# razayunus/ManhattanSLAM

Measured on AMD Instinct MI355X. Metric: RGB-D frames/sec at 640x480 (ORB+surfel front end), higher is better.
Workload: dtype u8/i32 (ORB)/f32+f64 (surfel)

## Files before the change

manhattanslam_amd/csrc/msl_sf.h:

```cpp
#pragma once

#include "msl_common.h"

#include <hip/hip_ext.h>

namespace msl {
namespace sf {

constexpr int SP = 8;
constexpr int NCHUNK = 10;
constexpr double MAX_ANGLE_COS = 0.1, HUBER_RANGE = 0.4, MIN_TOLERATE_DIFF = 0.1;
constexpr unsigned T_INF = 0xFFFFFFFFu;
constexpr int PROP_ROUNDS = 6;
constexpr unsigned short IDX_NONE = 0xFFFF, IDX_PLANE = 0xFFFE;
constexpr int LIST_D = 256;
constexpr int SCAN_ITEMS = 1024;
#ifndef MSL_SUB_ITEMS
#define MSL_SUB_ITEMS 128
#endif
constexpr int SUB_ITEMS = MSL_SUB_ITEMS;
constexpr int DEFER_WIN = 32;
#ifndef MSL_FUSEREC_PLANES
#define MSL_FUSEREC_PLANES 0
#endif
__host__ __device__ inline size_t fuserec_index(int nseeds, unsigned seed, int word) {
#if MSL_FUSEREC_PLANES
    return (size_t)word * (size_t)nseeds + seed;
#else
    (void)nseeds; return 3 * (size_t)seed + (size_t)word;
#endif
}

enum SfCtr {
    CTR_LIVE = 0,
    CTR_NEW = 1,
    CTR_DELETED = 2,
    CTR_UPDATED = 3,
    CTR_BEFORE = 4,
    CTR_ERR = 5,
    CTR_AFTER = 6,
    CTR_TAIL_FLAG = 7,
    CTR_SELECTED = 7,
    CTR_TOT_NEW = 8, CTR_TOT_DELETED = 9, CTR_TOT_UPDATED = 10, CTR_TOT_KF = 11, CTR_TOT_BEFORE = 12,
    CTR_WIDE = 13,
    CTR_COUNT = 16
};

struct alignas(16) HotPk { float px, py, pz; unsigned tl; };
struct HotRec { float px, py, pz; int updateTimes, lastUpdate; };
constexpr unsigned HOT_WIDE = 0x80000000u, HOT_HOLE = 0xFFFFFFFFu;
__host__ __device__ inline bool tl_fits(int ut, int lu) { return (unsigned)ut < 2048u && ((unsigned)lu + (1u << 19)) < (1u << 20); }
__host__ __device__ inline unsigned tl_pack(int ut, int lu) { return ((unsigned)ut << 20) | ((unsigned)lu & 0xFFFFFu); }
__host__ __device__ inline int tl_ut(unsigned tl) { return (int)(tl >> 20); }
__host__ __device__ inline int tl_lu(unsigned tl) { return (int)(tl << 12) >> 12; }
struct alignas(32) ColdRec { float nx, ny, nz, size, color, weight; unsigned rgbf; unsigned _spare; };
constexpr unsigned COLD_WIDE = 1u << 24;
struct MapSoA {
    HotPk *hot;
    ColdRec *cold;
    int *rgbWide;
    int *utlWide;
    long long *wideFlag;
};
__host__ __device__ inline bool rgb_fits(int r, int g, int b) { return ((unsigned)r | (unsigned)g | (unsigned)b) < 256u; }
__host__ __device__ inline unsigned rgb_pack(int r, int g, int b) { return (unsigned)r | ((unsigned)g << 8) | ((unsigned)b << 16); }

template <typename T> using gptr = const T __attribute__((address_space(1))) *;
struct FrameDev {
    const uint8_t *gray; const float *depth; const int32_t *member;
    float pose[16], invPose[16];
    int ref, _pad;
#ifdef __HIPCC__
    __device__ __forceinline__ gptr<uint8_t> grayG() const { return (gptr<uint8_t>)gray; }
    __device__ __forceinline__ gptr<float> depthG() const { return (gptr<float>)depth; }
    __device__ __forceinline__ gptr<int32_t> memberG() const { return (gptr<int32_t>)member; }
#endif
};

struct alignas(32) AssignRec {
    float x, y, meanIntensity;
    unsigned stable;
    double invDepth;
    unsigned long long _pad;
};

struct FuseAux {
    MapSoA map;
    unsigned long long cap;
    unsigned *delU, *delUCount;
    unsigned *delList;
};
struct DeferCtl {
    long long ext[DEFER_WIN + 1];
    unsigned delCnt[DEFER_WIN];
    unsigned logBase[DEFER_WIN];
    unsigned nMoves;
    int flagStride;
    const uint8_t *candOk, *fused;
    const msl_surfel *cand;
    FuseAux aux;
};

struct SfDev {
    int W, H, spW, spH, nseeds, npx;
    float fx, fy, cx, cy, fuseFar, fuseNear;
    unsigned long long gstride, gbytes, dstride, mstride;
    unsigned gsB, dsB, msB;
    const FrameDev *frames;
    msl_seed *seeds, *seedsTmp;
    msl_surfel *cand;
    uint8_t *candOk;
    uint8_t *fused;
    uint2 *tex;
    float4 *fuseRec;
    unsigned short *index, *amap;
    unsigned *tmin;
    AssignRec *arec;
    float *pxInv;
    unsigned *wl;
    unsigned *wlCount;
    int *chunkAbort;
    int *changed;
    MapSoA map;
    unsigned long long cap;
    long long *ctr;
    msl_surfel *newSurfels;
    unsigned *blockSums, *blockUpd, *delList, *srcOf;
    unsigned *sbKeys, *deal;
    int dealG;
    unsigned *tickets;
    unsigned *delU;
    unsigned *delUCount;
    const float *colX, *rowY;
    int pxStride;
    int flagStride;
    int kf;
    int prevSlotAbs;
    DeferCtl *dc;
    unsigned *moveDst;
    unsigned long long *loc64;
    unsigned *vposD;
    unsigned *locKeys, *vposKeys;
    unsigned *dBig;
    unsigned *bitmap;
    HotPk *stageHot; ColdRec *stageCold; int *stageRgb, *stageUtl;
};

#ifdef __HIPCC__
__device__ __forceinline__ AssignRec assign_rec(const msl_seed &s) {
    AssignRec a;
    a.x = s.x; a.y = s.y; a.meanIntensity = s.meanIntensity; a.stable = s.stable ? 1u : 0u;
    a.invDepth = s.meanDepth > 0 ? 1.0 / (double)s.meanDepth : -1.0; a._pad = 0;
    return a;
}
__device__ __forceinline__ int seed_chunk(int seedI, int nseeds) {
    const int step = nseeds / NCHUNK;
    if (step == 0) return NCHUNK - 1;
    const int c = seedI / step;
    return c > NCHUNK - 1 ? NCHUNK - 1 : c;
}
template <typename T> __device__ __forceinline__ gptr<T> byte_off(gptr<T> p, unsigned off) {
    return reinterpret_cast<gptr<T>>(reinterpret_cast<const char __attribute__((address_space(1))) *>(p) + off);
}
template <typename T> __device__ __forceinline__ gptr<T> byte_off(const T *p, unsigned off) { return byte_off((gptr<T>)p, off); }
template <typename T> using gptr_w = T __attribute__((address_space(1))) *;
template <typename T> __device__ __forceinline__ gptr_w<T> byte_off_w(T *p, unsigned off) {
    return reinterpret_cast<gptr_w<T>>(reinterpret_cast<char __attribute__((address_space(1))) *>((gptr_w<T>)p) + off);
}
__device__ __forceinline__ uint8_t gray_at(const SfDev &P, const FrameDev &F, int y, int x) { return *byte_off(F.grayG(), (unsigned)y * P.gsB + (unsigned)x); }
__device__ __forceinline__ float depth_at(const SfDev &P, const FrameDev &F, int y, int x) { return *byte_off(F.depthG(), (unsigned)y * P.dsB + 4u * (unsigned)x); }
__device__ __forceinline__ int32_t member_at(const SfDev &P, const FrameDev &F, int y, int x) {
    return *byte_off(F.memberG(), ((unsigned)y >> 1) * P.msB + 4u * ((unsigned)x >> 1));
}
__device__ __forceinline__ void vec3b(const SfDev &P, const FrameDev &F, float row, float col, int &r, int &g, int &b) {
    const unsigned long long off = (unsigned long long)(int)row * P.gstride + 3ull * (unsigned long long)(int)col;
    r = off < P.gbytes ? F.grayG()[off] : 0;
    g = off + 1 < P.gbytes ? F.grayG()[off + 1] : 0;
    b = off + 2 < P.gbytes ? F.grayG()[off + 2] : 0;
}
__device__ __forceinline__ void back_project(const SfDev &P, float u, float v, float d, float &x, float &y, float &z) {
    x = (u - P.cx) / P.fx * d;
    y = (v - P.cy) / P.fy * d;
    z = d;
}
__device__ __forceinline__ float get_weight(float d) { const double a = 1.0 / (double)d / (double)d; return (float)(1.0 < a ? 1.0 : a); }
__device__ __forceinline__ void mul4(const float *m, float v0, float v1, float v2, float v3, float out[4]) {
#pragma unroll
    for (int r = 0; r < 4; r++) out[r] = ((m[r] * v0 + m[4 + r] * v1) + m[8 + r] * v2) + m[12 + r] * v3;
}
__device__ __forceinline__ void mul3(const float *m, float v0, float v1, float v2, float out[3]) {
#pragma unroll
    for (int r = 0; r < 3; r++) out[r] = (m[r] * v0 + m[4 + r] * v1) + m[8 + r] * v2;
}
#endif

template <typename T>
__host__ __device__ inline void inverse4(const T *m, T *inv) {
#define M_(r, c) m[(c) * 4 + (r)]
#define DET3(r0, r1, r2, c0, c1, c2)                                                                     \
    (M_(r0, c0) * (M_(r1, c1) * M_(r2, c2) - M_(r1, c2) * M_(r2, c1)) -                                 \
     M_(r0, c1) * (M_(r1, c0) * M_(r2, c2) - M_(r1, c2) * M_(r2, c0)) +                                 \
     M_(r0, c2) * (M_(r1, c0) * M_(r2, c1) - M_(r1, c1) * M_(r2, c0)))
    T cof[4][4];
    for (int r = 0; r < 4; r++)
        for (int c = 0; c < 4; c++) {
            int rr[3], cc[3], k = 0;
            for (int i = 0; i < 4; i++) if (i != r) rr[k++] = i;
            k = 0;
            for (int i = 0; i < 4; i++) if (i != c) cc[k++] = i;
            const T d = DET3(rr[0], rr[1], rr[2], cc[0], cc[1], cc[2]);
            cof[r][c] = ((r + c) & 1) ? -d : d;
        }
    const T det = ((M_(0, 0) * cof[0][0] + M_(0, 1) * cof[0][1]) + M_(0, 2) * cof[0][2]) + M_(0, 3) * cof[0][3];
    for (int r = 0; r < 4; r++)
        for (int c = 0; c < 4; c++) inv[c * 4 + r] = cof[c][r] / det;
#undef DET3
#undef M_
}

#ifdef __HIPCC__
__device__ __forceinline__ bool xcd_slot(int blocksPerFrame, int nSlots, int &slot, int &blk) {
    const unsigned lin = blockIdx.x;
    const unsigned j = lin >> 3;
    slot = (int)(lin & 7u) + 8 * (int)(j / (unsigned)blocksPerFrame);
    blk = (int)(j % (unsigned)blocksPerFrame);
    return slot < nSlots;
}
#endif
inline unsigned xcd_grid(int blocksPerFrame, int nSlots) { return 8u * (unsigned)((nSlots + 7) / 8) * (unsigned)blocksPerFrame; }

enum { SK_SEED_INIT = 0, SK_ASSIGN, SK_PROP, SK_COMMIT_PX, SK_UPDATE_SEEDS, SK_COMMIT_SEEDS, SK_SEED_PLANE, SK_FUSE, SK_NEW, SK_COMPACT,
       SK_CONVERT, SK_COPY };

#define MSL_SF_LAUNCH_LDS(prof, kid, st, kern, grid, block, lds, ...)                                  \
    do {                                                                                               \
        hipEvent_t _ea, _eb;                                                                           \
        if ((prof).kernel_pair(kid, &_ea, &_eb))                                                       \
            hipExtLaunchKernelGGL(kern, grid, block, lds, st, _ea, _eb, 0, __VA_ARGS__);               \
        else                                                                                           \
            hipLaunchKernelGGL(kern, grid, block, lds, st, __VA_ARGS__);                               \
    } while (0)
#define MSL_SF_LAUNCH(prof, kid, st, kern, grid, block, ...) MSL_SF_LAUNCH_LDS(prof, kid, st, kern, grid, block, 0, __VA_ARGS__)

bool sp_init_attributes(int nseeds);
void sp_launch_stage(KernelProfiler &prof, hipStream_t st, const SfDev &P, int nFrames, bool propLds);
void sp_launch_depth_u16(hipStream_t st, const void *src, size_t srcStride, size_t srcFrameStride, float *dst, size_t dstFrameStride, int W, int H, int nFrames,
                         float factor);
int sp_debug_div100(const float *x_host, double *out_host, size_t n);
int sp_debug_chain(const float *x_host, const int32_t *n_host, int lists, int huber, float *out_host);
void map_launch_fuse(KernelProfiler &prof, hipStream_t st, const SfDev &P, int slot, const FrameDev &F, int nSubGrid, int nSubHint, bool deferred, bool dealt, unsigned blkStride);
void map_launch_compact(KernelProfiler &prof, hipStream_t st, const SfDev &P, int slot, bool resident);
void map_launch_deal(hipStream_t st, const SfDev &P);
int map_debug_deal(const uint32_t *keys_host, int G, uint32_t *deal_host);
void map_launch_replay(KernelProfiler &prof, hipStream_t st, const SfDev &P, int nFrames, unsigned blkStride);
void map_launch_empty_pair(KernelProfiler &prof, hipStream_t st);
void map_launch_set_ctr(hipStream_t st, const SfDev &P, long long n, int wide);
void map_launch_add_ctr(hipStream_t st, const SfDev &P, long long add);
void map_launch_aos_to_soa(KernelProfiler &prof, hipStream_t st, const SfDev &P, const msl_surfel *src, long long n, bool atEnd);
void map_launch_soa_to_aos(KernelProfiler &prof, hipStream_t st, const SfDev &P, msl_surfel *dst, long long n);
void map_launch_select_count(hipStream_t st, const SfDev &P, int mode, int arg);
void map_launch_select_write(hipStream_t st, const SfDev &P, int mode, int arg, msl_surfel *out, int markDeleted);
void map_launch_collect_changed(hipStream_t st, const SfDev &P, int ref, long long n, unsigned *count, unsigned *idxOut, msl_surfel *recOut, unsigned capOut);
void map_launch_empty(hipStream_t st, int grid, hipEvent_t a, hipEvent_t b);

}
}
```

manhattanslam_amd/csrc/msl_sf_sp_assign.hip:

```cpp

#include "msl_sf_sp_dev.h"

namespace {

__global__ __launch_bounds__(256) void kb_seed_init(SfDev P) {
    const int slot = blockIdx.y;
    const int seedI = blockIdx.x * 256 + threadIdx.x;
    if (seedI >= P.nseeds) return;
    if (seedI == 0) P.wlCount[slot] = 0;
    const FrameDev F = P.frames[slot];
    const int spX = seedI % P.spW, spY = seedI / P.spW;
    int imageX = spX * SP + SP / 2, imageY = spY * SP + SP / 2;
    imageX = imageX < (P.W - 1) ? imageX : (P.W - 1);
    imageY = imageY < (P.H - 1) ? imageY : (P.H - 1);
    msl_seed s;
    memset(&s, 0, sizeof(s));
    P.fused[(size_t)slot * P.flagStride + seedI] = 0;
    if (member_at(P, F, imageY, imageX) != -1) {
        P.seeds[(size_t)slot * P.nseeds + seedI] = s; P.arec[(size_t)slot * P.nseeds + seedI] = assign_rec(s);
        return;
    }
    s.use = 1;
    s.x = (float)imageX; s.y = (float)imageY;
    vec3b(P, F, (float)imageY, (float)imageX, s.r, s.g, s.b);
    s.meanIntensity = gray_at(P, F, imageY, imageX);
    s.meanDepth = depth_at(P, F, imageY, imageX);
    if (s.meanDepth < 0.01) {
        int xb = spX * SP + SP / 2 - SP, yb = spY * SP + SP / 2 - SP;
        int xe = xb + SP * 2, ye = yb + SP * 2;
        xb = xb > 0 ? xb : 0; yb = yb > 0 ? yb : 0;
        xe = xe < P.W - 1 ? xe : P.W - 1; ye = ye < P.H - 1 ? ye : P.H - 1;
        bool found = false;
        for (int j = yb; j < ye && !found; j++)
            for (int i = xb; i < xe; i++) {
                const float d = depth_at(P, F, j, i);
                if (d > 0.01) { s.meanDepth = d; found = true; break; }
            }
    }
    P.seeds[(size_t)slot * P.nseeds + seedI] = s;
    P.arec[(size_t)slot * P.nseeds + seedI] = assign_rec(s);
}

constexpr int ASSIGN_NY = 2;
__global__ __launch_bounds__(256) void kb_assign(SfDev P, int it, int nSlots, int nbx, int nby) {
    const int bpr = (nbx + 3) >> 2;
    const int nbyG = (nby + ASSIGN_NY - 1) / ASSIGN_NY;
    int slot, blk;
    if (!xcd_slot(bpr * nbyG, nSlots, slot, blk)) return;
    if (blk == 0) {
        if (it > 0 && threadIdx.x < 8) P.changed[slot * 8 + threadIdx.x] = threadIdx.x == 0 ? 1 : 0;
        if (threadIdx.x >= 64 && threadIdx.x < 64 + NCHUNK) P.chunkAbort[(slot * 2 + (it & 1)) * 16 + threadIdx.x - 64] = 0x7FFFFFFF;
    }
    const int wv = __builtin_amdgcn_readfirstlane((int)(threadIdx.x >> 6));
    const int byg = blk / bpr, bxi = (blk - byg * bpr) * 4 + wv;
    if (bxi >= nbx) return;
    const int bx = bxi - 1, by0 = byg * ASSIGN_NY - 1;
    const bool okx0 = bx >= 0 && bx < P.spW, okx1 = bx + 1 < P.spW;
    const int bxc = min(bx, P.spW - 1);
    const AssignRec *arec = P.arec + (unsigned)slot * (unsigned)P.nseeds;
    AssignRec cr[ASSIGN_NY + 1][2];
    int rowIdx[ASSIGN_NY + 1];
#pragma unroll
    for (int r = 0; r <= ASSIGN_NY; r++) {
        const int rc = min(max(by0 + r, 0), P.spH - 1);
        rowIdx[r] = rc * P.spW + bx;
        const AssignRec *rp = arec + (rc * P.spW + bxc);
        cr[r][0] = rp[0]; cr[r][1] = rp[1];
    }
    const FrameDev F = P.frames[slot];
    unsigned short *index = P.index + (size_t)slot * P.pxStride, *amap = P.amap + (size_t)slot * P.pxStride;
    float *pxInv = P.pxInv + (size_t)slot * P.pxStride;
    unsigned *tmin = P.tmin + (size_t)slot * P.nseeds;
    const int lane = threadIdx.x & 63, lx = lane & 7, ly = lane >> 3;
    const int colI = 8 * bx + 4 + lx;
    const float colF = (float)colI;
    const bool colIn = colI >= 0 && colI < P.W;
    bool inImg[ASSIGN_NY];
    int mem[ASSIGN_NY], cur[ASSIGN_NY];
    float gI[ASSIGN_NY], dIn[ASSIGN_NY];
    unsigned tCur[ASSIGN_NY];
#pragma unroll
    for (int k = 0; k < ASSIGN_NY; k++) {
        const int rowI = 8 * (by0 + k) + 4 + ly;
        inImg[k] = colIn && rowI >= 0 && rowI < P.H && by0 + k + 1 < nby;
        const int rowC = min(max(rowI, 0), P.H - 1), colC = min(max(colI, 0), P.W - 1), pc = rowC * P.W + colC;
        mem[k] = member_at(P, F, rowC, colC);
        gI[k] = gray_at(P, F, rowC, colC);
        dIn[k] = it == 0 ? depth_at(P, F, rowC, colC) : *byte_off(pxInv, 4u * (unsigned)pc);
        cur[k] = it == 0 ? 0 : (int)*byte_off(index, 2u * (unsigned)pc);
    }
#pragma unroll
    for (int k = 0; k < ASSIGN_NY; k++)
        tCur[k] = it == 0 ? 0u : *byte_off(tmin, 4u * (unsigned)cur[k]);
#pragma unroll
    for (int k = 0; k < ASSIGN_NY; k++) {
        const int by = by0 + k;
        if (__ballot(inImg[k]) == 0) continue;
        const bool oky0 = by >= 0 && by < P.spH, oky1 = by + 1 < P.spH;
        const int rowI = 8 * by + 4 + ly;
        const int p = rowI * P.W + colI;
        const bool isPlane = mem[k] != -1;
        const float myIntensity = gI[k];
        float myInvDepth = dIn[k];
        if (it == 0) {
            myInvDepth = 0.0f;
            if (dIn[k] > 0.01) myInvDepth = (float)(1.0 / (double)dIn[k]);
            if (inImg[k] && !isPlane) *byte_off_w(pxInv, 4u * (unsigned)p) = myInvDepth;
        }
        const bool pxHasDepth = myInvDepth > 0;
        const double myInvD = (double)myInvDepth;
        const float rowF = (float)rowI;
        float minDistDepth = 1e6f, minDistNodepth = 1e6f;
        int minSpIndexDepth = -1, minSpIndexNodepth = -1;
        bool allHasDepth = true;
        auto consider = [&](const AssignRec &C, int spIndex, bool use) {
            float nodepthCost = 0;
            const float dist = (C.x - colF) * (C.x - colF) + (C.y - rowF) * (C.y - rowF);
            nodepthCost += dist / ((SP / 2) * (SP / 2));
            const float intensityDiff = C.meanIntensity - myIntensity;
            nodepthCost = (float)((double)nodepthCost + div100_exact((double)(intensityDiff * intensityDiff)));
            const bool has = C.invDepth >= 0 && pxHasDepth;
            const float inverseDepthDiff = (float)(C.invDepth - myInvD);
            const float withDepth = (float)((double)nodepthCost + (double)(inverseDepthDiff * inverseDepthDiff) * 400.0);
            const float depthCost = has ? withDepth : nodepthCost;
            allHasDepth = allHasDepth && (has || !use);
            const bool bd = use && depthCost < minDistDepth, bn = use && nodepthCost < minDistNodepth;
            minDistDepth = bd ? depthCost : minDistDepth; minSpIndexDepth = bd ? spIndex : minSpIndexDepth;
            minDistNodepth = bn ? nodepthCost : minDistNodepth; minSpIndexNodepth = bn ? spIndex : minSpIndexNodepth;
        };
        const bool anyStable = (cr[k][0].stable | cr[k][1].stable | cr[k + 1][0].stable | cr[k + 1][1].stable) != 0;
        if (okx0 && oky0) consider(cr[k][0], rowIdx[k], true);
        if (okx0 && oky1) consider(cr[k + 1][0], rowIdx[k + 1], ly != 0);
        if (okx1 && oky0) consider(cr[k][1], rowIdx[k] + 1, lx != 0);
        if (okx1 && oky1) consider(cr[k + 1][1], rowIdx[k + 1] + 1, lx != 0 && ly != 0);
        const int pick = allHasDepth ? minSpIndexDepth : minSpIndexNodepth;
        if (!inImg[k]) continue;
        if (it == 0) { *byte_off_w(index, 2u * (unsigned)p) = isPlane ? (unsigned short)0 : (unsigned short)(pick >= 0 ? pick : 0); continue; }
        *byte_off_w(amap, 2u * (unsigned)p) = isPlane ? IDX_PLANE : (pick >= 0 ? (unsigned short)pick : IDX_NONE);
        if (!isPlane && pick >= 0) {
            if (tCur[k] == 0) {
                if (anyStable && tmin[pick] > (unsigned)p + 1u) atomicMin(&tmin[pick], (unsigned)p + 1u);
            } else if (pick != cur[k]) {
                P.wl[(size_t)slot * P.pxStride + atomicAdd(&P.wlCount[slot], 1u)] = (unsigned)p;
            }
        }
    }
}

__device__ __forceinline__ bool relax_pixel(unsigned *tmin, const unsigned short *index, const unsigned short *amap, int p) {
    const unsigned short a = amap[p];
    if (a >= IDX_PLANE) return false;
    const unsigned tc = __hip_atomic_load(&tmin[index[p]], __ATOMIC_RELAXED, __HIP_MEMORY_SCOPE_AGENT);
    if (tc == 0 || tc > (unsigned)p) return false;
    if (__hip_atomic_load(&tmin[a], __ATOMIC_RELAXED, __HIP_MEMORY_SCOPE_AGENT) <= (unsigned)p + 1u) return false;
    return atomicMin(&tmin[a], (unsigned)p + 1u) > (unsigned)p + 1u;
}

constexpr int PROP_BLOCKS = 16;
__global__ __launch_bounds__(256) void kb_prop(SfDev P, int round, int nSlots) {
    int slot, blk;
    if (!xcd_slot(PROP_BLOCKS, nSlots, slot, blk)) return;
    if (!P.changed[slot * 8 + round]) return;
    unsigned *tmin = P.tmin + (size_t)slot * P.nseeds;
    const unsigned short *index = P.index + (size_t)slot * P.pxStride, *amap = P.amap + (size_t)slot * P.pxStride;
    const unsigned *wl = P.wl + (size_t)slot * P.pxStride;
    const unsigned nwl = P.wlCount[slot];
    bool any = false;
    for (unsigned e = blk * 256 + threadIdx.x; e < nwl; e += PROP_BLOCKS * 256) any |= relax_pixel(tmin, index, amap, (int)wl[e]);
    if (any) P.changed[slot * 8 + round + 1] = 1;
}

__global__ __launch_bounds__(1024) void kb_prop_finish(SfDev P) {
    __shared__ int s_ch;
    const int slot = blockIdx.x;
    if (threadIdx.x == 0) s_ch = P.changed[slot * 8 + PROP_ROUNDS];
    __syncthreads();
    unsigned *tmin = P.tmin + (size_t)slot * P.nseeds;
    const unsigned short *index = P.index + (size_t)slot * P.pxStride, *amap = P.amap + (size_t)slot * P.pxStride;
    const unsigned *wl = P.wl + (size_t)slot * P.pxStride;
    const unsigned nwl = P.wlCount[slot];
    while (s_ch) {
        __syncthreads();
        if (threadIdx.x == 0) s_ch = 0;
        __syncthreads();
        bool any = false;
        for (unsigned e = threadIdx.x; e < nwl; e += 1024) any |= relax_pixel(tmin, index, amap, (int)wl[e]);
        if (any) s_ch = 1;
        __syncthreads();
    }
}

constexpr int PROP_LDS_MAX_SEEDS = 36 * 1024;
__global__ __launch_bounds__(256) void kb_prop_lds(SfDev P) {
    extern __shared__ unsigned s_t[];
    const int slot = blockIdx.x;
    const unsigned nwl = P.wlCount[slot];
    if (nwl == 0) return;
    unsigned *tmin = P.tmin + (size_t)slot * P.nseeds;
    const unsigned short *index = P.index + (size_t)slot * P.pxStride, *amap = P.amap + (size_t)slot * P.pxStride;
    const unsigned *wl = P.wl + (size_t)slot * P.pxStride;
    constexpr int NT = 256, R = 16;
    unsigned ep[R];
    unsigned short ec[R], ea[R];
#pragma unroll
    for (int r = 0; r < R; r++) {
        const unsigned e = threadIdx.x + r * NT;
        ep[r] = 0xFFFFFFFFu; ec[r] = 0; ea[r] = 0;
        if (e < nwl) { const unsigned p = wl[e]; ep[r] = p; ec[r] = index[p]; ea[r] = amap[p]; }
    }
    for (int i = threadIdx.x; i < P.nseeds; i += NT) s_t[i] = tmin[i];
    __syncthreads();
    auto relax = [&](unsigned p, unsigned short cur, unsigned short a) -> bool {
        if (a >= IDX_PLANE) return false;
        const unsigned tc = s_t[cur];
        if (tc == 0 || tc > p) return false;
        if (s_t[a] <= p + 1u) return false;
        return atomicMin(&s_t[a], p + 1u) > p + 1u;
    };
    int any;
    do {
        bool ch = false;
#pragma unroll
        for (int r = 0; r < R; r++)
            if (ep[r] != 0xFFFFFFFFu) ch |= relax(ep[r], ec[r], ea[r]);
        for (unsigned e = threadIdx.x + R * NT; e < nwl; e += NT) { const unsigned p = wl[e]; ch |= relax(p, index[p], amap[p]); }
        any = __syncthreads_or(ch ? 1 : 0);
    } while (any);
    for (int i = threadIdx.x; i < P.nseeds; i += NT) {
        const unsigned t = s_t[i];
        if (t != tmin[i]) tmin[i] = t;
    }
}

__global__ __launch_bounds__(256) void kb_commit_px(SfDev P, int nSlots) {
    int slot, blk;
    if (!xcd_slot(((P.npx + 7) / 8 + 255) / 256, nSlots, slot, blk)) return;
    const int p0 = (blk * 256 + threadIdx.x) * 8;
    if (p0 >= P.npx) return;
    unsigned short *index = P.index + (size_t)slot * P.pxStride;
    const uint4 a4 = *reinterpret_cast<const uint4 *>(P.amap + (size_t)slot * P.pxStride + p0);
    uint4 i4 = *reinterpret_cast<const uint4 *>(index + p0);
    const unsigned *tmin = P.tmin + (size_t)slot * P.nseeds;
    unsigned aw[4] = {a4.x, a4.y, a4.z, a4.w}, iw[4] = {i4.x, i4.y, i4.z, i4.w};
    bool changed = false;
#pragma unroll
    for (int k = 0; k < 8; k++) {
        const unsigned a = (aw[k >> 1] >> (16 * (k & 1))) & 0xFFFFu, cur = (iw[k >> 1] >> (16 * (k & 1))) & 0xFFFFu;
        if (a >= IDX_PLANE || a == cur || p0 + k >= P.npx) continue;
        if (tmin[cur] <= (unsigned)(p0 + k)) {
            iw[k >> 1] = (iw[k >> 1] & ~(0xFFFFu << (16 * (k & 1)))) | (a << (16 * (k & 1)));
            changed = true;
        }
    }
    if (changed) { i4.x = iw[0]; i4.y = iw[1]; i4.z = iw[2]; i4.w = iw[3]; *reinterpret_cast<uint4 *>(index + p0) = i4; }
}

__global__ void k_debug_div100(const float *x, double *out, long long n) {
    const long long i = (long long)blockIdx.x * 256 + threadIdx.x;
    if (i < n) out[i] = div100_exact((double)(x[i] * x[i]));
}

}

namespace msl {
namespace sf {

bool sp_init_attributes(int nseeds) {
    if (nseeds > PROP_LDS_MAX_SEEDS) return false;
    return hipFuncSetAttribute((const void *)kb_prop_lds, hipFuncAttributeMaxDynamicSharedMemorySize, (int)(sizeof(unsigned) * PROP_LDS_MAX_SEEDS)) == hipSuccess;
}

void sp_launch_seed_init(KernelProfiler &prof, hipStream_t sp, const SfDev &P, int n) {
    MSL_SF_LAUNCH(prof, SK_SEED_INIT, sp, kb_seed_init, sp_seed_grid(P, n), dim3(256), P);
}

void sp_launch_pixel_pass(KernelProfiler &prof, hipStream_t sp, const SfDev &P, int n, int it, bool propLds) {
    const int W = P.W, H = P.H;
    const unsigned un = (unsigned)n;
    const int nbx = ((W - 5) >> 3) + 2, nby = ((H - 5) >> 3) + 2;
    const dim3 pxGrid(xcd_grid(((nbx + 3) / 4) * ((nby + ASSIGN_NY - 1) / ASSIGN_NY), n)), flatPx(xcd_grid(((P.npx + 7) / 8 + 255) / 256, n));
    MSL_SF_LAUNCH(prof, SK_ASSIGN, sp, kb_assign, pxGrid, dim3(256), P, it, n, nbx, nby);
    if (it > 0) {
        prof.begin(SK_PROP, sp);
        if (propLds) {
            hipLaunchKernelGGL(kb_prop_lds, dim3(un), dim3(256), sizeof(unsigned) * P.nseeds, sp, P);
        } else {
            for (int r = 0; r < PROP_ROUNDS; r++) hipLaunchKernelGGL(kb_prop, dim3(xcd_grid(PROP_BLOCKS, n)), dim3(256), 0, sp, P, r, n);
            hipLaunchKernelGGL(kb_prop_finish, dim3(un), dim3(1024), 0, sp, P);
        }
        prof.end(sp);
        MSL_SF_LAUNCH(prof, SK_COMMIT_PX, sp, kb_commit_px, flatPx, dim3(256), P, n);
    }
}

int sp_debug_div100(const float *x_host, double *out_host, size_t n) {
    if (n == 0) return MSL_OK;
    if (!x_host || !out_host) return MSL_ERR_INVALID;
    DevBuf x, out;
    MSL_HIP_TRY(grow_all(0, {{x, sizeof(float) * n}, {out, sizeof(double) * n}}));
    MSL_HIP_TRY(hipMemcpy(x.p, x_host, sizeof(float) * n, hipMemcpyHostToDevice));
    hipLaunchKernelGGL(k_debug_div100, dim3((unsigned)((n + 255) / 256)), dim3(256), 0, 0, (const float *)x.p, (double *)out.p, (long long)n);
    MSL_HIP_TRY(hipMemcpy(out_host, out.p, sizeof(double) * n, hipMemcpyDeviceToHost));
    return MSL_OK;
}

}
}
```

manhattanslam_amd/csrc/msl_sf_sp_seeds.hip:

```cpp

#include "msl_sf_sp_dev.h"

namespace {

struct SeedUpd {
    int state;
    int cnt, sumI, sumX, sumY;
    int depthLoop;
    float meanDepth;
};
static_assert(sizeof(SeedUpd) <= sizeof(msl_seed), "the hand-over record fits a seedsTmp record");
template <bool STRADDLE>
__global__ __launch_bounds__(256) void kb_update_seeds(SfDev P, int it, int nSlots) {
    __shared__ __attribute__((aligned(16))) float s_depth[16][272];
    int slot, blk;
    if (!xcd_slot((P.nseeds + 15) / 16, nSlots, slot, blk)) return;
#ifdef MSL_FUSE_STAMPS
    unsigned long long ust[8]; int usn = 0;
#define USTAMP() ust[usn++] = __builtin_amdgcn_s_memtime()
#else
#define USTAMP()
#endif
    USTAMP();
    const int g = threadIdx.x >> 4, l = threadIdx.x & 15;
    const int seedI = blk * 16 + g;
    const FrameDev F = P.frames[slot];
    const unsigned short *index = P.index + (size_t)slot * P.pxStride;
    msl_seed S;
    memset(&S, 0, sizeof(S));
    bool active = seedI < P.nseeds;
    bool stable = false;
    if (active) {
        S = P.seeds[(size_t)slot * P.nseeds + seedI];
        stable = it > 0 ? (P.tmin[(size_t)slot * P.nseeds + seedI] == T_INF) : (S.stable != 0);
        if (!S.use || stable) {
            if (l == 0) {
                P.seeds[(size_t)slot * P.nseeds + seedI].stable = stable;
                P.arec[(size_t)slot * P.nseeds + seedI].stable = stable ? 1u : 0u;
                reinterpret_cast<SeedUpd *>(P.seedsTmp + ((size_t)slot * P.nseeds + seedI))->state = 0;
                P.tmin[(size_t)slot * P.nseeds + seedI] = stable ? T_INF : 0u;
            }
            active = false;
        }
    }
    if (!__ballot(active)) return;
    const int spX = seedI % P.spW, spY = seedI / P.spW;
    const int xb0 = spX * SP + SP / 2 - SP, yb0 = spY * SP + SP / 2 - SP;
    const int xb = xb0 > 0 ? xb0 : 0, yb = yb0 > 0 ? yb0 : 0;
    const int xe = (xb0 + SP * 2) < P.W - 1 ? (xb0 + SP * 2) : P.W - 1, ye = (yb0 + SP * 2) < P.H - 1 ? (yb0 + SP * 2) : P.H - 1;
    int sumX = 0, sumY = 0, sumI = 0, cnt = 0, nd = 0;
    {
        const int rq = l >> 2, cq = l & 3;
        const int col0 = xb0 + 4 * cq;
        const bool quadIn = col0 >= 0 && (STRADDLE ? col0 < P.W : col0 + 3 < P.W);
        const int colc = quadIn ? (STRADDLE ? min(col0, P.W - 4) : col0) : 0;
        Quad<unsigned short> idq[4];
        Quad<float> dq[4];
        Quad<uint8_t> gq[4];
#pragma unroll
        for (int m = 0; m < 4; m++) {
            const int jc = min(max(yb0 + 4 * m + rq, 0), P.H - 1);
            idq[m] = load_quad(byte_off(index, 2u * (unsigned)(jc * P.W + colc)));
            dq[m] = load_quad(byte_off(F.depthG(), (unsigned)jc * P.dsB + 4u * (unsigned)colc));
            gq[m] = load_quad(byte_off(F.grayG(), (unsigned)jc * P.gsB + (unsigned)colc));
        }
#pragma unroll
        for (int m = 0; m < 4; m++) {
            const int j = yb0 + 4 * m + rq;
            const bool rowOk = active && quadIn && j >= yb && j < ye;
            bool hd[4];
            int c = 0;
#pragma unroll
            for (int e = 0; e < 4; e++) {
                const int col = colc + e;
                const bool own = rowOk && (!STRADDLE || col >= col0) && col >= xb && col < xe && idq[m].v[e] == seedI;
                hd[e] = own && dq[m].v[e] >= DEPTH_01_F;
                if (own) { sumX += col; sumY += j; sumI += gq[m].v[e]; cnt++; }
                c += hd[e] ? 1 : 0;
            }
            const int incl = row_incl_scan(c);
            int o = nd + incl - c;
#pragma unroll
            for (int e = 0; e < 4; e++)
                if (hd[e]) s_depth[g][o++] = dq[m].v[e];
            nd += row_lane_i32<15>(incl);
        }
    }
    USTAMP();
    sumX = row_sum_i32(sumX); sumY = row_sum_i32(sumY); sumI = row_sum_i32(sumI); cnt = row_sum_i32(cnt);
    __builtin_amdgcn_wave_barrier();
    const bool depthLoop = active && cnt != 0 && nd > 0;
    if (l == 0 && active && cnt == 0)
        atomicMin(&P.chunkAbort[(slot * 2 + (it & 1)) * 16 + seed_chunk(seedI, P.nseeds)], seedI);
    const int ndL = depthLoop ? nd : 0;
    const int nblk = rows_max_i32((ndL + 15) >> 4);
    float meanDepth = 0.0f;
    {
        float sd = 0.0f;
        for (int bq = 0; bq < nblk; bq++) {
            const int e = l + 16 * bq;
            sd = chain_block_f32(sd, e < ndL ? s_depth[g][e] : 0.0f);
        }
        const float sumDepth = row_lane_f32<15>(sd);
        if (depthLoop) meanDepth = sumDepth / (float)nd;
    }
    USTAMP();
    bool open = depthLoop;
    for (int newtonI = 0; newtonI < 5; newtonI++) {
        if (!__ballot(open)) break;
        int inr = 0;
        bool tail = false;
        for (int bq = 0; bq < nblk; bq++) {
            const int e = l + 16 * bq;
            if (open && e < ndL) {
                const float residual = meanDepth - s_depth[g][e];
                if (in_huber_band(residual)) inr++; else tail = true;
            }
        }
        inr = row_sum_i32(inr);
        const bool anyTail = __ballot(tail) != 0ull;
        float sa = 0.0f;
        for (int bq = 0; bq < nblk; bq++) {
            const int e = l + 16 * bq;
            float t = 0.0f;
            if (open && e < ndL) {
                const float residual = meanDepth - s_depth[g][e];
                if (in_huber_band(residual)) t = 2 * residual;
                else t = residual > 0 ? __builtin_inff() : -__builtin_inff();
            }
            sa = anyTail ? chain_block_huber(sa, t) : chain_block_f32(sa, t);
        }
        const float sumA = row_lane_f32<15>(sa);
        const float sumB = (float)(2 * inr);
        const float deltaDepth = (float)((double)(-sumA) / ((double)sumB + 10.0));
        if (open) {
            meanDepth = meanDepth + deltaDepth;
            if ((deltaDepth < 0.01 && deltaDepth > -0.01) || newtonI == 4) open = false;
        }
    }
    USTAMP();
    if (active && l == 0) {
        SeedUpd U;
        U.state = cnt == 0 ? 1 : 2; U.cnt = cnt; U.sumI = sumI; U.sumX = sumX; U.sumY = sumY; U.depthLoop = depthLoop ? 1 : 0; U.meanDepth = meanDepth;
        *reinterpret_cast<SeedUpd *>(P.seedsTmp + ((size_t)slot * P.nseeds + seedI)) = U;
    }
#ifdef MSL_FUSE_STAMPS
    USTAMP();
    if (slot == 0 && (threadIdx.x & 63) == 0) {
        for (int q = 1; q < usn; q++) atomicAdd(&P.delList[96 + q], (unsigned)(ust[q] - ust[q - 1]));
        atomicAdd(&P.delList[96], 1u);
    }
#endif
}

__global__ __launch_bounds__(256) void kb_commit_seeds(SfDev P, int it) {
    const int slot = blockIdx.y;
    const int seedI = blockIdx.x * 256 + threadIdx.x;
    if (seedI >= P.nseeds) return;
    if (seedI == 0) P.wlCount[slot] = 0;
    const size_t si = (size_t)slot * P.nseeds + seedI;
    const SeedUpd U = *reinterpret_cast<const SeedUpd *>(P.seedsTmp + si);
    if (U.state == 0) return;
    const int abortAt = P.chunkAbort[(slot * 2 + (it & 1)) * 16 + seed_chunk(seedI, P.nseeds)];
    if (U.state == 1 || seedI > abortAt) {
        P.seeds[si].stable = 0; P.arec[si].stable = 0u; P.tmin[si] = 0u;
        return;
    }
    const FrameDev &F = P.frames[slot];
    static_assert(sizeof(msl_seed) == 64 && offsetof(msl_seed, meanDepth) == 40 && offsetof(msl_seed, r) == 48 && offsetof(msl_seed, stable) == 61, "msl_seed layout");
    uint4 *rec = reinterpret_cast<uint4 *>(P.seeds + si);
    const uint4 w0o = rec[0], w2o = rec[2], w3o = rec[3];
    const float sumIntensityNum = (float)U.cnt;
    const float sumIntensity = (float)U.sumI / sumIntensityNum, mX = (float)U.sumX / sumIntensityNum, mY = (float)U.sumY / sumIntensityNum;
    const float preIntensity = __uint_as_float(w2o.w), preX = __uint_as_float(w0o.x), preY = __uint_as_float(w0o.y);
    int tR = 0, tG = 0, tB = 0;
    vec3b(P, F, mY, mX, tR, tG, tB);
    const float updateDiff = fabsf(preIntensity - sumIntensity) + fabsf(preX - mX) + fabsf(preY - mY);
    const bool tStable = updateDiff < 0.2;
    const float tDepth = U.depthLoop ? U.meanDepth : 0.0f;
    uint4 w0 = w0o, w2 = w2o, w3 = w3o;
    w0.x = __float_as_uint(mX); w0.y = __float_as_uint(mY);
    w2.z = __float_as_uint(tDepth); w2.w = __float_as_uint(sumIntensity);
    w3.x = (unsigned)tR; w3.y = (unsigned)tG; w3.z = (unsigned)tB;
    w3.w = (w3.w & 0x00FF00FFu) | (tStable ? 0x100u : 0u);
    rec[0] = w0; rec[2] = w2; rec[3] = w3;
    P.tmin[si] = tStable ? T_INF : 0u;
    AssignRec a;
    a.x = mX; a.y = mY; a.meanIntensity = sumIntensity; a.stable = tStable ? 1u : 0u;
    a.invDepth = tDepth > 0 ? 1.0 / (double)tDepth : -1.0; a._pad = 0;
    P.arec[si] = a;
}

__global__ __launch_bounds__(64) void k_debug_chain(const float *x, const int *n, float *out, int lists, int huber) {
    const int q = blockIdx.x * 4 + (threadIdx.x >> 4), l = threadIdx.x & 15;
    const int nq = q < lists ? n[q] : 0;
    int nblk = (nq + 15) >> 4;
#pragma unroll
    for (int d = 32; d >= 16; d >>= 1) nblk = max(nblk, __shfl_xor(nblk, d, 64));
    nblk = __builtin_amdgcn_readfirstlane(nblk);
    float s = 0.0f;
    for (int bq = 0; bq < nblk; bq++) {
        const int e = l + 16 * bq;
        const float t = e < nq ? x[(size_t)q * 256 + e] : 0.0f;
        s = huber ? chain_block_huber(s, t) : chain_block_f32(s, t);
    }
    if (q < lists && l == 15) out[q] = s;
}

}

namespace msl {
namespace sf {

void sp_launch_seed_pass(KernelProfiler &prof, hipStream_t sp, const SfDev &P, int n, int it) {
    if (sp_quad_straddles(P.W)) MSL_SF_LAUNCH(prof, SK_UPDATE_SEEDS, sp, kb_update_seeds<true>, dim3(xcd_grid((P.nseeds + 15) / 16, n)), dim3(256), P, it, n);
    else MSL_SF_LAUNCH(prof, SK_UPDATE_SEEDS, sp, kb_update_seeds<false>, dim3(xcd_grid((P.nseeds + 15) / 16, n)), dim3(256), P, it, n);
    MSL_SF_LAUNCH(prof, SK_COMMIT_SEEDS, sp, kb_commit_seeds, sp_seed_grid(P, n), dim3(256), P, it);
}

int sp_debug_chain(const float *x_host, const int32_t *n_host, int lists, int huber, float *out_host) {
    if (lists <= 0) return MSL_OK;
    if (!x_host || !n_host || !out_host) return MSL_ERR_INVALID;
    for (int q = 0; q < lists; q++) if (n_host[q] < 0 || n_host[q] > 256) return MSL_ERR_INVALID;
    DevBuf x, cnt, out;
    MSL_HIP_TRY(grow_all(0, {{x, sizeof(float) * 256 * (size_t)lists}, {cnt, sizeof(int) * (size_t)lists}, {out, sizeof(float) * (size_t)lists}}));
    MSL_HIP_TRY(hipMemcpy(x.p, x_host, sizeof(float) * 256 * (size_t)lists, hipMemcpyHostToDevice));
    MSL_HIP_TRY(hipMemcpy(cnt.p, n_host, sizeof(int) * (size_t)lists, hipMemcpyHostToDevice));
    hipLaunchKernelGGL(k_debug_chain, dim3((unsigned)((lists + 3) / 4)), dim3(64), 0, 0, (const float *)x.p, (const int *)cnt.p, (float *)out.p, lists, huber);
    MSL_HIP_TRY(hipMemcpy(out_host, out.p, sizeof(float) * (size_t)lists, hipMemcpyDeviceToHost));
    return MSL_OK;
}

}
}
```

Before: 26830.

## Retile assign rows, cache Newton depth blocks in registers, sign-bit depth test

Each assign block now covers three superpixel rows instead of two, so more neighbour records are reused per load and fewer blocks are launched. The chunkAbort init moves to threads 32..41. In the seed update, the first four 16-wide depth blocks are kept in registers across Newton iterations, and their residual terms are cached too, which cuts repeated LDS reads. The candidate depth test becomes a scalar sign-bit check on the high word of invDepth. These are separate ideas; the taller tile raises register pressure and may lower occupancy.

```diff
diff --git a/manhattanslam_amd/csrc/msl_sf.h b/manhattanslam_amd/csrc/msl_sf.h
--- a/manhattanslam_amd/csrc/msl_sf.h
+++ b/manhattanslam_amd/csrc/msl_sf.h
@@ -83,6 +83,13 @@
     double invDepth;
     unsigned long long _pad;
 };
+constexpr double arec_inv_depth(float meanDepth) { return meanDepth > 0 ? 1.0 / (double)meanDepth : -1.0; }
+static_assert(arec_inv_depth(0.0f) == -1.0 && arec_inv_depth(-0.0f) == -1.0 && arec_inv_depth(-2.5f) == -1.0 && arec_inv_depth(__builtin_nanf("")) == -1.0,
+              "no valid depth: the literal -1.0");
+static_assert(__builtin_bit_cast(unsigned long long, arec_inv_depth(__builtin_inff())) == 0ull && arec_inv_depth(2.0f) == 0.5 &&
+              arec_inv_depth(__builtin_bit_cast(float, 1u)) > 0 && arec_inv_depth(__builtin_bit_cast(float, 1u)) < 1e46,
+              "a valid depth: sign bit clear from +inf (+0.0) down to the smallest denormal (finite)");
+static_assert((__builtin_bit_cast(unsigned long long, -1.0) >> 63) == 1ull, "-1.0 has its sign bit set");
 
 struct FuseAux {
     MapSoA map;
@@ -150,8 +157,13 @@
 __device__ __forceinline__ AssignRec assign_rec(const msl_seed &s) {
     AssignRec a;
     a.x = s.x; a.y = s.y; a.meanIntensity = s.meanIntensity; a.stable = s.stable ? 1u : 0u;
-    a.invDepth = s.meanDepth > 0 ? 1.0 / (double)s.meanDepth : -1.0; a._pad = 0;
+    a.invDepth = arec_inv_depth(s.meanDepth); a._pad = 0;
     return a;
+}
+__device__ __forceinline__ bool arec_has_depth(const AssignRec &C) {
+    int hi = (int)(__builtin_bit_cast(unsigned long long, C.invDepth) >> 32);
+    asm("" : "+s"(hi));
+    return hi >= 0;
 }
 __device__ __forceinline__ int seed_chunk(int seedI, int nseeds) {
     const int step = nseeds / NCHUNK;
diff --git a/manhattanslam_amd/csrc/msl_sf_sp_assign.hip b/manhattanslam_amd/csrc/msl_sf_sp_assign.hip
--- a/manhattanslam_amd/csrc/msl_sf_sp_assign.hip
+++ b/manhattanslam_amd/csrc/msl_sf_sp_assign.hip
@@ -41,18 +41,19 @@
     P.arec[(size_t)slot * P.nseeds + seedI] = assign_rec(s);
 }
 
-constexpr int ASSIGN_NY = 2;
-__global__ __launch_bounds__(256) void kb_assign(SfDev P, int it, int nSlots, int nbx, int nby) {
-    const int bpr = (nbx + 3) >> 2;
-    const int nbyG = (nby + ASSIGN_NY - 1) / ASSIGN_NY;
+constexpr int ASSIGN_NY = 3;
+constexpr int ASSIGN_WAVES = 4;
+__host__ __device__ constexpr int assign_blocks(int nbx, int nby) { return ((nbx + ASSIGN_WAVES - 1) / ASSIGN_WAVES) * ((nby + ASSIGN_NY - 1) / ASSIGN_NY); }
+__global__ __launch_bounds__(64 * ASSIGN_WAVES) void kb_assign(SfDev P, int it, int nSlots, int nbx, int nby) {
+    const int bpr = (nbx + ASSIGN_WAVES - 1) / ASSIGN_WAVES;
     int slot, blk;
-    if (!xcd_slot(bpr * nbyG, nSlots, slot, blk)) return;
+    if (!xcd_slot(assign_blocks(nbx, nby), nSlots, slot, blk)) return;
     if (blk == 0) {
         if (it > 0 && threadIdx.x < 8) P.changed[slot * 8 + threadIdx.x] = threadIdx.x == 0 ? 1 : 0;
-        if (threadIdx.x >= 64 && threadIdx.x < 64 + NCHUNK) P.chunkAbort[(slot * 2 + (it & 1)) * 16 + threadIdx.x - 64] = 0x7FFFFFFF;
+        if (threadIdx.x >= 32 && threadIdx.x < 32 + NCHUNK) P.chunkAbort[(slot * 2 + (it & 1)) * 16 + threadIdx.x - 32] = 0x7FFFFFFF;
     }
     const int wv = __builtin_amdgcn_readfirstlane((int)(threadIdx.x >> 6));
-    const int byg = blk / bpr, bxi = (blk - byg * bpr) * 4 + wv;
+    const int byg = blk / bpr, bxi = (blk - byg * bpr) * ASSIGN_WAVES + wv;
     if (bxi >= nbx) return;
     const int bx = bxi - 1, by0 = byg * ASSIGN_NY - 1;
     const bool okx0 = bx >= 0 && bx < P.spW, okx1 = bx + 1 < P.spW;
@@ -114,12 +115,13 @@
         int minSpIndexDepth = -1, minSpIndexNodepth = -1;
         bool allHasDepth = true;
         auto consider = [&](const AssignRec &C, int spIndex, bool use) {
+            const bool candHas = arec_has_depth(C);
             float nodepthCost = 0;
             const float dist = (C.x - colF) * (C.x - colF) + (C.y - rowF) * (C.y - rowF);
             nodepthCost += dist / ((SP / 2) * (SP / 2));
             const float intensityDiff = C.meanIntensity - myIntensity;
             nodepthCost = (float)((double)nodepthCost + div100_exact((double)(intensityDiff * intensityDiff)));
-            const bool has = C.invDepth >= 0 && pxHasDepth;
+            const bool has = candHas && pxHasDepth;
             const float inverseDepthDiff = (float)(C.invDepth - myInvD);
             const float withDepth = (float)((double)nodepthCost + (double)(inverseDepthDiff * inverseDepthDiff) * 400.0);
             const float depthCost = has ? withDepth : nodepthCost;
@@ -278,8 +280,8 @@
     const int W = P.W, H = P.H;
     const unsigned un = (unsigned)n;
     const int nbx = ((W - 5) >> 3) + 2, nby = ((H - 5) >> 3) + 2;
-    const dim3 pxGrid(xcd_grid(((nbx + 3) / 4) * ((nby + ASSIGN_NY - 1) / ASSIGN_NY), n)), flatPx(xcd_grid(((P.npx + 7) / 8 + 255) / 256, n));
-    MSL_SF_LAUNCH(prof, SK_ASSIGN, sp, kb_assign, pxGrid, dim3(256), P, it, n, nbx, nby);
+    const dim3 pxGrid(xcd_grid(assign_blocks(nbx, nby), n)), flatPx(xcd_grid(((P.npx + 7) / 8 + 255) / 256, n));
+    MSL_SF_LAUNCH(prof, SK_ASSIGN, sp, kb_assign, pxGrid, dim3(64 * ASSIGN_WAVES), P, it, n, nbx, nby);
     if (it > 0) {
         prof.begin(SK_PROP, sp);
         if (propLds) {
diff --git a/manhattanslam_amd/csrc/msl_sf_sp_seeds.hip b/manhattanslam_amd/csrc/msl_sf_sp_seeds.hip
--- a/manhattanslam_amd/csrc/msl_sf_sp_seeds.hip
+++ b/manhattanslam_amd/csrc/msl_sf_sp_seeds.hip
@@ -10,11 +10,14 @@
     float meanDepth;
 };
 static_assert(sizeof(SeedUpd) <= sizeof(msl_seed), "the hand-over record fits a seedsTmp record");
+constexpr int UPD_SEEDS = 16;
+constexpr int NEWTON_RB = 4;
+__host__ __device__ constexpr int upd_blocks(int nseeds) { return (nseeds + UPD_SEEDS - 1) / UPD_SEEDS; }
 template <bool STRADDLE>
-__global__ __launch_bounds__(256) void kb_update_seeds(SfDev P, int it, int nSlots) {
-    __shared__ __attribute__((aligned(16))) float s_depth[16][272];
+__global__ __launch_bounds__(16 * UPD_SEEDS) void kb_update_seeds(SfDev P, int it, int nSlots) {
+    __shared__ __attribute__((aligned(16))) float s_depth[UPD_SEEDS][272];
     int slot, blk;
-    if (!xcd_slot((P.nseeds + 15) / 16, nSlots, slot, blk)) return;
+    if (!xcd_slot(upd_blocks(P.nseeds), nSlots, slot, blk)) return;
 #ifdef MSL_FUSE_STAMPS
     unsigned long long ust[8]; int usn = 0;
 #define USTAMP() ust[usn++] = __builtin_amdgcn_s_memtime()
@@ -23,7 +26,7 @@
 #endif
     USTAMP();
     const int g = threadIdx.x >> 4, l = threadIdx.x & 15;
-    const int seedI = blk * 16 + g;
+    const int seedI = blk * UPD_SEEDS + g;
     const FrameDev F = P.frames[slot];
     const unsigned short *index = P.index + (size_t)slot * P.pxStride;
     msl_seed S;
@@ -95,9 +98,19 @@
     const int ndL = depthLoop ? nd : 0;
     const int nblk = rows_max_i32((ndL + 15) >> 4);
     float meanDepth = 0.0f;
+    float dr[NEWTON_RB > 0 ? NEWTON_RB : 1], tr[NEWTON_RB > 0 ? NEWTON_RB : 1];
     {
         float sd = 0.0f;
-        for (int bq = 0; bq < nblk; bq++) {
+#pragma unroll
+        for (int bq = 0; bq < NEWTON_RB; bq++) {
+            dr[bq] = 0.0f;
+            if (bq < nblk) {
+                const int e = l + 16 * bq;
+                dr[bq] = e < ndL ? s_depth[g][e] : 0.0f;
+                sd = chain_block_f32(sd, dr[bq]);
+            }
+        }
+        for (int bq = NEWTON_RB; bq < nblk; bq++) {
             const int e = l + 16 * bq;
             sd = chain_block_f32(sd, e < ndL ? s_depth[g][e] : 0.0f);
         }
@@ -110,7 +123,16 @@
         if (!__ballot(open)) break;
         int inr = 0;
         bool tail = false;
-        for (int bq = 0; bq < nblk; bq++) {
+#pragma unroll
+        for (int bq = 0; bq < NEWTON_RB; bq++) {
+            tr[bq] = 0.0f;
+            if (bq < nblk && open && l + 16 * bq < ndL) {
+                const float residual = meanDepth - dr[bq];
+                if (in_huber_band(residual)) { inr++; tr[bq] = 2 * residual; }
+                else { tail = true; tr[bq] = residual > 0 ? __builtin_inff() : -__builtin_inff(); }
+            }
+        }
+        for (int bq = NEWTON_RB; bq < nblk; bq++) {
             const int e = l + 16 * bq;
             if (open && e < ndL) {
                 const float residual = meanDepth - s_depth[g][e];
@@ -120,7 +142,10 @@
         inr = row_sum_i32(inr);
         const bool anyTail = __ballot(tail) != 0ull;
         float sa = 0.0f;
-        for (int bq = 0; bq < nblk; bq++) {
+#pragma unroll
+        for (int bq = 0; bq < NEWTON_RB; bq++)
+            if (bq < nblk) sa = anyTail ? chain_block_huber(sa, tr[bq]) : chain_block_f32(sa, tr[bq]);
+        for (int bq = NEWTON_RB; bq < nblk; bq++) {
             const int e = l + 16 * bq;
             float t = 0.0f;
             if (open && e < ndL) {
@@ -187,7 +212,7 @@
     P.tmin[si] = tStable ? T_INF : 0u;
     AssignRec a;
     a.x = mX; a.y = mY; a.meanIntensity = sumIntensity; a.stable = tStable ? 1u : 0u;
-    a.invDepth = tDepth > 0 ? 1.0 / (double)tDepth : -1.0; a._pad = 0;
+    a.invDepth = arec_inv_depth(tDepth); a._pad = 0;
     P.arec[si] = a;
 }
 
@@ -213,8 +238,8 @@
 namespace sf {
 
 void sp_launch_seed_pass(KernelProfiler &prof, hipStream_t sp, const SfDev &P, int n, int it) {
-    if (sp_quad_straddles(P.W)) MSL_SF_LAUNCH(prof, SK_UPDATE_SEEDS, sp, kb_update_seeds<true>, dim3(xcd_grid((P.nseeds + 15) / 16, n)), dim3(256), P, it, n);
-    else MSL_SF_LAUNCH(prof, SK_UPDATE_SEEDS, sp, kb_update_seeds<false>, dim3(xcd_grid((P.nseeds + 15) / 16, n)), dim3(256), P, it, n);
+    if (sp_quad_straddles(P.W)) MSL_SF_LAUNCH(prof, SK_UPDATE_SEEDS, sp, kb_update_seeds<true>, dim3(xcd_grid(upd_blocks(P.nseeds), n)), dim3(16 * UPD_SEEDS), P, it, n);
+    else MSL_SF_LAUNCH(prof, SK_UPDATE_SEEDS, sp, kb_update_seeds<false>, dim3(xcd_grid(upd_blocks(P.nseeds), n)), dim3(16 * UPD_SEEDS), P, it, n);
     MSL_SF_LAUNCH(prof, SK_COMMIT_SEEDS, sp, kb_commit_seeds, sp_seed_grid(P, n), dim3(256), P, it);
 }
 
```

Measured after the change: 27150 (median of 6 runs). +1.2%, better.
